# interstellar/zkvm

Hardware: AMD Instinct MI355X
Metric: ZkVM tx verifications/sec (batch) (higher is better)
Workload: dtype u32 limb pairs of radix-2^51 (v_mad_u64_u32)

## Files before the change

### zkvm_amd/csrc/kernels.hpp

```cpp
#pragma once
#include "curve.hpp"
#include "quad.hpp"
#include "sc_dev.hpp"

namespace zk {

constexpr uint32_t ENTRY_NEG = 1u << 31;
constexpr uint32_t ENTRY_DYN = 1u << 30;
constexpr uint32_t ENTRY_IDX = (1u << 30) - 1;
constexpr int NIELS_WORDS = 32;
constexpr int EXT_WORDS = 40;
constexpr int REDUCE_CHUNK = 64;
#ifndef ZK_REDUCE_CHUNK_BIG
#define ZK_REDUCE_CHUNK_BIG 16
#endif
constexpr int REDUCE_CHUNK_BIG = ZK_REDUCE_CHUNK_BIG;
constexpr int TABLE_WORDS = 24;
constexpr int TABLE_STRIDE = 32;

struct JobDesc {
  const uint32_t* dyn_scalars;
  const uint64_t* dyn_offsets;
  uint64_t n_dyn;
  const uint32_t* st_scalars;
// ... 871 lines not shown
  fe_mul(c4.T, p.T, fe_D2());
  store_ext(row, c4);
}

__global__ void __launch_bounds__(64)
k_small_tables(const uint32_t* __restrict__ dyn_scalars, const uint32_t* __restrict__ dyn_rows, uint64_t n,
               uint32_t* __restrict__ tbl , uint32_t* __restrict__ recoded ,
               uint32_t* __restrict__ status) {
  const uint64_t k = (uint64_t)blockIdx.x * 64 + threadIdx.x;
  if (k >= n) return;
  if (dyn_scalars) {
    const uint32_t* sc = dyn_scalars + 8 * k;
    if (sc[7] >> 31) atomicOr(&status[0], 2u);
    uint32_t carry = 0;
#pragma unroll
    for (int i = 0; i < 8; ++i) {
      const uint64_t v = (uint64_t)sc[i] + 0x88888888u + carry;
      recoded[8 * k + i] = (uint32_t)v;
      carry = (uint32_t)(v >> 32);
    }
  }
  ge_niels nq;
  load_niels(nq, dyn_rows + k * NIELS_WORDS);
  ge cur;
  ge_identity(cur);
  uint32_t* row = tbl + k * (SMALL_TBL * EXT_WORDS);
#pragma unroll 1
  for (int e = 0; e < SMALL_TBL; ++e) {
    ge_madd(cur, cur, nq, false);
    store_cached(row + e * EXT_WORDS, cur);
  }
}

__global__ void __launch_bounds__(256)
k_small_accumulate(const uint32_t* __restrict__ recoded, const uint64_t* __restrict__ dyn_offsets,
                   const uint32_t* __restrict__ tbl, uint32_t n_msm, uint32_t* __restrict__ window_sums,
                   uint32_t* __restrict__ window_nonempty) {
  extern __shared__ __attribute__((aligned(16))) uint32_t smem[];
  const uint32_t m = blockIdx.x;
  const int t = threadIdx.x & 63;
  const int part = threadIdx.x >> 6, parts = blockDim.x >> 6;
  const uint64_t k0 = dyn_offsets[m], k1 = dyn_offsets[m + 1];
  ge total;
  bool total_set = false;
#pragma unroll 1
  for (uint64_t k = k0 + part; k < k1; k += parts) {
    const uint32_t n4 = (recoded[8 * k + (t >> 3)] >> (4 * (t & 7))) & 15u;
    const int d = (t == 63 && n4 < 8u) ? (int)n4 + 8 : (int)n4 - 8;
    if (d != 0) {
      ge c4;
      load_ext(c4, tbl + (k * SMALL_TBL + (uint64_t)((d < 0 ? -d : d) - 1)) * EXT_WORDS);
      ge_cached c;
      c.YpX = c4.X; c.YmX = c4.Y; c.Z2 = c4.Z; c.T2d = c4.T;
      if (!total_set) { ge_identity(total); total_set = true; }
      ge_add_cached(total, total, c, d < 0);
    }
  }
  if (part > 0) {
    uint32_t* slot = smem + (uint32_t)(part - 1) * 41 * 64;
    slot[40 * 64 + t] = total_set ? 1u : 0u;
    if (total_set) {
#pragma unroll
      for (int q = 0; q < 10; ++q) {
        slot[q * 64 + t] = total.X.v[q]; slot[(10 + q) * 64 + t] = total.Y.v[q];
        slot[(20 + q) * 64 + t] = total.Z.v[q]; slot[(30 + q) * 64 + t] = total.T.v[q];
      }
    }
  }
  __syncthreads();
  if (part != 0) return;
#pragma unroll 1
  for (int o = 1; o < parts; ++o) {
    const uint32_t* slot = smem + (uint32_t)(o - 1) * 41 * 64;
    if (slot[40 * 64 + t]) {
      ge other;
#pragma unroll
      for (int q = 0; q < 10; ++q) {
        other.X.v[q] = slot[q * 64 + t]; other.Y.v[q] = slot[(10 + q) * 64 + t];
        other.Z.v[q] = slot[(20 + q) * 64 + t]; other.T.v[q] = slot[(30 + q) * 64 + t];
      }
      if (total_set) ge_add(total, total, other); else { total = other; total_set = true; }
    }
  }
  const uint64_t win = (uint64_t)m * 64 + t;
  window_nonempty[win] = total_set ? 1u : 0u;
  if (total_set) store_ext(window_sums + win * EXT_WORDS, total);
}

__global__ void __launch_bounds__(256)
k_msm_finish_quad(const uint32_t* __restrict__ window_sums, const uint32_t* __restrict__ window_nonempty,
                  const uint32_t* __restrict__ msm_fail, uint8_t* __restrict__ accept,
                  uint32_t* __restrict__ out_enc, uint32_t* __restrict__ out_ext, uint32_t n_msm, int w,
                  int n_windows, const uint32_t* __restrict__ sel_state, uint32_t sel_group) {
  const uint32_t g = blockIdx.x * blockDim.x + threadIdx.x;
  const int r = g & 3;
  const bool live = (g >> 2) < n_msm;
  const uint32_t m = live ? (g >> 2) : (n_msm - 1);
  if (sel_state && sel_state[m / sel_group] == 0) return;
  ge acc;
  ge_identity(acc);
  bool have = false;
  const uint64_t win0 = (uint64_t)m * n_windows;
  ge p;
  uint32_t ne = window_nonempty[win0 + n_windows - 1];
  load_ext(p, window_sums + (win0 + n_windows - 1) * EXT_WORDS);
  for (int t = n_windows - 1; t >= 0; --t) {
    ge pn;
    uint32_t nen = 0;
    if (t > 0) {
      nen = window_nonempty[win0 + t - 1];
      load_ext(pn, window_sums + (win0 + t - 1) * EXT_WORDS);
    }
    if (have) {
      for (int k = 0; k < w; ++k) quad_double(acc, r);
    }
    if (ne) {
      if (have) quad_add(acc, p, r); else { acc = p; have = true; }
    }
    if (t > 0) { p = pn; ne = nen; }
// ... 135 lines not shown
    ge_niels nq;
    niels_from_affine(nq, x, y);
    store_table_row(myrows + (uint64_t)d * TABLE_STRIDE, nq);
  }
}

__global__ void __launch_bounds__(256)
k_static_digits(const uint32_t* __restrict__ st_scalars, int16_t* __restrict__ digits, uint64_t n_static, int w,
                int W, uint32_t* __restrict__ status, const uint32_t* __restrict__ row_map ,
                const uint32_t* __restrict__ n_active , uint32_t rows_per_msm, uint32_t fold_small_negatives) {
  uint64_t k = (uint64_t)blockIdx.x * blockDim.x + threadIdx.x;
  if (k >= n_static) return;
  if (row_map) {
    const uint32_t slot = (uint32_t)(k / rows_per_msm);
    if (slot >= *n_active) return;
    k = (uint64_t)row_map[slot] * rows_per_msm + k % rows_per_msm;
  }
  const uint32_t* sc = st_scalars + 8 * k;
  if (sc[7] >> 31) atomicOr(&status[0], 2u);
  for (int t = 0; t < W; ++t) digits[(uint64_t)t * n_static + k] = 0;
  if (fold_small_negatives) {
    const uint32_t l[8] = ZK_SC_L;
    uint32_t v[8];
    uint64_t br = 0;
    for (int i = 0; i < 8; ++i) { const uint64_t d = (uint64_t)l[i] - sc[i] - br; v[i] = (uint32_t)d; br = (d >> 32) & 1; }
    uint32_t high = v[0] >> 14;
    for (int i = 1; i < 8; ++i) high |= v[i];
    if (br == 0 && high == 0 && v[0] != 0 && w >= 15) { digits[k] = (int16_t)(-(int)v[0]); return; }
  }
  for_each_digit(sc, w, W, [&](int t, int d) { digits[(uint64_t)t * n_static + k] = (int16_t)d; });
}

template <bool kSkipZeros>
__global__ void __launch_bounds__(256)
k_static_accumulate(const int16_t* __restrict__ digits, const uint64_t* __restrict__ st_offsets,
                    const uint32_t* __restrict__ st_index, const uint32_t* __restrict__ table, uint32_t n_set,
                    uint32_t H, int W, int P, uint32_t n_msm, uint64_t n_static, uint32_t* __restrict__ partials,
                    const uint32_t* __restrict__ row_map ,
                    const uint32_t* __restrict__ n_active ,
                    uint32_t interleave ) {
  const uint64_t lane = (uint64_t)blockIdx.x * blockDim.x + threadIdx.x;
  if (lane >= (uint64_t)n_msm * W * P) return;
  const uint32_t part = (uint32_t)(lane % P);
  uint32_t slot = (uint32_t)((lane / P) % n_msm);
  const uint32_t t = (uint32_t)(lane / ((uint64_t)P * n_msm));
  if (n_active && slot >= *n_active) return;
  if (interleave > 1) { const uint32_t per = n_msm / interleave; slot = (slot % per) * interleave + slot / per; }
  const uint32_t tx = row_map ? row_map[slot] : slot;
  const uint64_t k0 = st_offsets[tx], k1 = st_offsets[tx + 1];
  const int16_t* dig = digits + (uint64_t)t * n_static;
  const uint64_t tbase = (uint64_t)t * n_set;
  ge acc;
  ge_identity(acc);
  auto fetch = [&](uint64_t k, ge_niels& q, bool& neg, bool& any) {
    int d = dig[k];
    d = (d == -32768) ? 32768 : d;
    any = d != 0;
    const uint32_t idx = st_index ? st_index[k] : (uint32_t)(k - k0);
    const uint32_t mag = (uint32_t)(d < 0 ? -d : d);
    if (!kSkipZeros || any) load_table_row(q, table + ((tbase + idx) * H + (mag ? mag - 1 : 0)) * TABLE_STRIDE);
    if (!any) niels_identity(q);
    neg = d < 0;
  };
  uint64_t k = k0 + part;
  ge_niels cur, nxt;
  bool cur_neg = false, nxt_neg = false, cur_any = false, nxt_any = false;
  if (k < k1) fetch(k, cur, cur_neg, cur_any);
  while (k < k1) {
    const uint64_t kn = k + P;
    if (kn < k1) fetch(kn, nxt, nxt_neg, nxt_any);
    if (!kSkipZeros || __any(cur_any)) ge_madd(acc, acc, cur, cur_neg);
    cur = nxt; cur_neg = nxt_neg; cur_any = nxt_any;
    k = kn;
  }
  store_ext(partials + (((uint64_t)slot * W + t) * P + part) * EXT_WORDS, acc);
}

__device__ inline void static_combine_slot(const uint32_t* __restrict__ partials, uint32_t n_partials, const uint32_t* __restrict__ dyn_sum,
                                           const uint8_t* __restrict__ dyn_ok, uint32_t slot, uint32_t tx, int lane,
                                           uint8_t* __restrict__ accept, uint32_t* __restrict__ out_points) {
  ge acc;
  ge_identity(acc);
  for (uint32_t c = lane; c < n_partials; c += 64) {
    ge p;
    load_ext(p, partials + ((uint64_t)slot * n_partials + c) * EXT_WORDS);
    ge_add(acc, acc, p);
  }
  if (lane == 0 && dyn_sum) {
    ge p;
    load_ext(p, dyn_sum + (uint64_t)tx * EXT_WORDS);
    ge_add(acc, acc, p);
  }
#pragma unroll 1
  for (int delta = 32; delta >= 1; delta >>= 1) {
    ge other;
    shfl_down_ge(other, acc, delta);
    if (lane < delta) ge_add(acc, acc, other);
  }
  if (lane == 0) {
    accept[tx] = (ge_is_identity(acc) && (!dyn_ok || dyn_ok[tx])) ? 1 : 0;
    if (out_points) store_ext(out_points + (uint64_t)slot * EXT_WORDS, acc);
  }
}

constexpr uint32_t COMBINE_LANES = 8;

__global__ void __launch_bounds__(64)
k_static_combine(const uint32_t* __restrict__ partials, uint32_t n_partials, const uint32_t* __restrict__ dyn_sum,
                 const uint8_t* __restrict__ dyn_ok, const uint32_t* __restrict__ row_map,
                 const uint32_t* __restrict__ n_active, uint32_t n_slots, uint8_t* __restrict__ accept,
// ... 518 lines not shown
```

### zkvm_amd/csrc/zkgpu.hip

```cpp
#include "../../include/zkgpu.h"
#include "../../include/zkgpu_hooks.h"
#include "kernels.hpp"
#include "keccak.hpp"

#include <hip/hip_runtime.h>

#include <algorithm>
#include <chrono>
#include <cerrno>
#include <cstdio>
#include <cstring>
#include <functional>
#include <memory>
#include <mutex>
#include <string>
#include <map>
#include <atomic>
#include <dirent.h>
#include <sys/random.h>
#include <unistd.h>
#include <thread>
#include <type_traits>
#include <vector>

// ... 66 lines not shown
  int sync_rc = 0, reasons_src = 0;
  std::recursive_mutex mu;
  std::string last_error;
  Buffer in_scalars, in_points, in_offsets, in_st_scalars, in_st_index, in_st_offsets;
  Buffer dyn_rows, bins, block_sums, entries, buckets, partials, partial_flags, window_sums, window_flags;
  Buffer msm_fail, status, accept, bitmap, ok_bytes, values, uniform;
  Buffer digits, st_partials, dynsum, accept2, bin_order, class_count, part_hist, part_entries, part_lo, dec_scratch, heavy;
  Buffer small_tbl, recoded;
  Buffer grp_sc, grp_digits, grp_partials, grp_ok, row_map;
  Buffer grp_ws, grp_wf, grp_dyn;
  Buffer grp_fail, grp_fail_sum, rechk_pts;
  struct LastBatch { bool valid = false, has_prep = false; const zkgpu_pointset* ps = nullptr; std::vector<uint8_t> job, prep; bool mixed = false; uint64_t mx_groups = 0, mx_stmts = 0; } last;
  bool force_unresolved = false;
  uint64_t regroup_fallbacks = 0, mx_stats[4] = {0, 0, 0, 0};
  int group_size = 16;
  bool serial = false;
  int horner_mode = 0;
  std::atomic<uint32_t> last_failed_groups{0};
  hipEvent_t ev_dig = nullptr, ev_u = nullptr;
  Buffer prep_com, prep_proofs, prep_r, prep_pw, prep_ch, prep_wf, prep_dyn_sc, prep_dyn_pt, prep_st_sc;
  Buffer coal_com, coal_proofs, coal_r, tx_reason;
  Buffer ipa_lv, ipa_rv, ipa_cg, ipa_ch, ipa_w, ipa_u;
  Buffer pv_plan, pv_state, pv_in, pv_rows0, pv_rows1, pv_rows2, pv_rows3, pv_lay, pv_pts, pv_com, pv_ab, pv_proofs;
  int prover_mode = 0;
  int prover_slices = 0;
  std::vector<zkgpu_ctx*> pv_slices;
  std::vector<uint32_t> pv_plan_host;
  size_t pv_lay_batch = 0;
  Buffer prep_absorb, prep_raw, mx_tab, mx_st_index, prep_large, mx_grp_index;
  int locate_mode = 0;
  int transcript_mode = 0;
  int forced_parts = 0;
  int locate_parts = 0;
  int tail_mode = 0;
  void* pinned = nullptr;
  size_t pinned_cap = 0;
  void* pinned_in = nullptr;
  size_t pinned_in_cap = 0;
  bool profiling = false;
  std::vector<ProfEntry> prof;
  std::vector<std::pair<hipEvent_t, hipEvent_t>> ev_pool;
  std::vector<std::pair<int, int>> ev_used;
  size_t ev_next = 0;
  int forced_w = 0, last_w = 0;
  DecodeRoutes decode_routes;
  uint64_t last_adds = 0, tx_hashed_on_device = 0, tx_signed_on_device = 0;
};

namespace {
void quiesce_after_fault(zkgpu_ctx* c) {
  zk::fault::Suppress open;
  int prev = -1;
  (void)hipGetDevice(&prev);
  if (prev != c->device) (void)hipSetDevice(c->device);
  if (hipDeviceSynchronize() != hipSuccess) c->broken = true;
  (void)hipGetLastError();
  if (prev >= 0 && prev != c->device) (void)hipSetDevice(prev);
}

#define HIP_TRY(ctx, expr)                                                                  \
  do {                                                                                      \
    if ((ctx)->broken) {                                                                    \
      (ctx)->last_error = "an earlier device fault on this context could not be drained: the context is unusable"; \
      return ZKGPU_EHIP;                                                                    \
    }                                                                                       \
    hipError_t e__ = (expr);                                                                \
    if (e__ != hipSuccess) {                                                                \
// ... 622 lines not shown
  return pipe_tables(c, ps) && pipe_rows_fit(n_msm, n_dyn, n_static);
}

int pipe_enqueue(zkgpu_ctx* c, const Job& job, const zkgpu_pointset* ps, const PrepLaunch* prep) {
  static_assert(std::is_trivially_copyable<Job>::value && std::is_trivially_copyable<PrepLaunch>::value, "kept as bytes");
  {
    std::vector<uint8_t> jb(sizeof(Job)), pb(prep ? sizeof(PrepLaunch) : 0);
    memcpy(jb.data(), &job, sizeof(Job));
    if (prep) memcpy(pb.data(), prep, sizeof(PrepLaunch));
    c->last.job.swap(jb); c->last.prep.swap(pb);
    c->last.ps = ps; c->last.has_prep = prep != nullptr; c->last.valid = true; c->last.mixed = false;
  }
  const size_t B = job.n_msm;
  const size_t nbytes = (B + 7) / 8;
  hipStream_t L = c->stream_l, H1 = c->serial ? L : c->stream, H2 = c->serial ? L : c->stream2;
  const hipStream_t H3s = c->serial ? L : c->stream3;
  const int W = ps->tbl_W;
  int P = c->forced_parts;
  if (P <= 0) {
    P = (int)((131072 + B * W - 1) / (B * W));
    P = std::max(1, std::min(16, P));
  }
  const uint64_t n_lanes = (uint64_t)B * W * P;
  const uint32_t group = (prep && c->group_size > 1) ? (uint32_t)std::min<size_t>(c->group_size, B) : 1;
  const uint32_t n_groups = (uint32_t)((B + group - 1) / group);
  const uint32_t ns = prep ? prep->plan.sh.n_static : 0;
  const bool locate = group > 1 && (c->locate_mode >= 2 || (c->locate_mode == 0 && B >= LOCATE_MIN_BATCH));
  const bool spec = locate && c->locate_mode == 3;
  const uint32_t grp_rows = spec ? 2 * n_groups : n_groups;
  int Pg = 1;
  const int Pf = 32;
  const int Pl = c->locate_parts > 0 ? c->locate_parts : 32;
  if (group > 1) {
    Pg = (int)std::max<uint64_t>(1, std::min<uint64_t>(32, (65536 + (uint64_t)grp_rows * W - 1) / ((uint64_t)grp_rows * W)));
    TRY(ensure(c, c->grp_sc, (size_t)grp_rows * ns * 32));
    TRY(ensure(c, c->grp_digits, (size_t)grp_rows * ns * W * 2));
    TRY(ensure(c, c->grp_partials, (size_t)grp_rows * std::max<size_t>((size_t)W * std::max(Pg, locate && !spec ? Pl : 0), TAIL_THREADS) * EXT_WORDS * 4));
    TRY(ensure(c, c->grp_ok, n_groups));
    TRY(ensure(c, c->row_map, B * 4));
    TRY(ensure(c, c->grp_fail, (size_t)n_groups * 12));
    TRY(ensure(c, c->grp_fail_sum, (size_t)n_groups * EXT_WORDS * 4));
    TRY(ensure(c, c->grp_ws, (size_t)n_groups * 64 * EXT_WORDS * 4));
    TRY(ensure(c, c->grp_wf, (size_t)n_groups * 64 * 4));
    TRY(ensure(c, c->grp_dyn, (size_t)n_groups * EXT_WORDS * 4));
    TRY(ensure(c, c->rechk_pts, B * EXT_WORDS * 4));
  }
  TRY(ensure(c, c->accept, B));
  TRY(ensure(c, c->accept2, B));
  TRY(ensure(c, c->bitmap, nbytes));
  TRY(ensure_pinned(c, nbytes + 64 + (c->want_reasons ? B : 0)));
  TRY(ensure(c, c->status, 64));
  TRY(ensure(c, c->digits, std::max<uint64_t>(job.n_static, 1) * W * 2));
  TRY(ensure(c, c->st_partials, std::max<uint64_t>(n_lanes, group > 1 ? (uint64_t)B * std::max(W * Pf, TAIL_THREADS) : 0) * EXT_WORDS * 4));
  TRY(ensure(c, c->dynsum, B * EXT_WORDS * 4));
  TRY(ensure(c, c->dyn_rows, std::max<uint64_t>(job.n_dyn, 1) * NIELS_WORDS * 4));
  TRY(ensure(c, c->window_sums, (size_t)B * 64 * EXT_WORDS * 4));
  TRY(ensure(c, c->window_flags, (size_t)B * 64 * 4));
  TRY(ensure(c, c->msm_fail, (size_t)B * 4));
  TRY(ensure(c, c->small_tbl, std::max<uint64_t>(job.n_dyn, 1) * SMALL_TBL * EXT_WORDS * 4));
  TRY(ensure(c, c->recoded, std::max<uint64_t>(job.n_dyn, 1) * 32));
  c->last_w = 4;
  if (c->reserve_only) return ZKGPU_OK;
  const int phase = prep ? c->enqueue_phase : (int)zkgpu_ctx::ENQ_ALL;
  if (phase == zkgpu_ctx::ENQ_ALL || phase == zkgpu_ctx::ENQ_FRONT) {
  {
    Launch l(c, "k_batch_init", L);
    hipLaunchKernelGGL(k_batch_init, dim3(blocks_for(B, 256)), dim3(256), 0, L, (uint32_t*)c->status.p,
// ... 26 lines not shown
        hipLaunchKernelGGL(k_challenges, dim3((unsigned)B), dim3(128), (size_t)sh.n_ch * 32, L, sh, (const uint32_t*)c->prep_raw.p,
                           (const uint32_t*)c->prep_pw.p, prep->d_r, (uint32_t)B, (uint32_t*)c->prep_ch.p,
                           (uint32_t*)c->prep_wf.p, d.mono_chal, d.mono_pow, group > 1 ? 1u : 0u);
      }
    } else {
      Launch l(c, "k_transcript", L);
      hipLaunchKernelGGL(k_transcript, dim3(blocks_for(B, 64)), dim3(64), 0, L, sh, d.init, d.tape, d.n_ops, prep->d_com,
                         (const uint32_t*)c->prep_pw.p, prep->d_r, (uint32_t)B, (uint32_t*)c->prep_ch.p,
                         (uint32_t*)c->prep_wf.p, d.mono_chal, d.mono_pow, group > 1 ? 1u : 0u);
    }
  }
  HIP_TRY(c, hipEventRecord(c->ev_t, L));
  }
  if (phase == zkgpu_ctx::ENQ_FRONT) { HIP_TRY(c, hipGetLastError()); c->awaiting_back = true; return ZKGPU_OK; }
  if (prep && (phase == zkgpu_ctx::ENQ_ALL || phase == zkgpu_ctx::ENQ_MID)) {
    const PrepShape& sh = prep->plan.sh;
    HIP_TRY(c, hipStreamWaitEvent(H1, c->ev_u, 0));
    {
      Launch l(c, "k_points_tables", H1);
      hipLaunchKernelGGL(k_points_tables, dim3(blocks_for((uint64_t)B * sh.n_dyn, 256)), dim3(256), 0, H1, sh,
                         prep->d_com, (const uint32_t*)c->prep_pw.p, (uint32_t)B, (uint32_t*)c->small_tbl.p,
                         (uint32_t*)c->msm_fail.p, (unsigned long long*)((char*)c->status.p + 8));
    }
    HIP_TRY(c, hipEventRecord(c->ev_dig, H1));
  }
  if (phase == zkgpu_ctx::ENQ_MID) { HIP_TRY(c, hipGetLastError()); return ZKGPU_OK; }
  c->awaiting_back = false;
  if (prep) {
    HIP_TRY(c, hipStreamWaitEvent(H3s, c->ev_t, 0));
    TRY(prepare_launch(c, H3s, *prep, (uint32_t)B, false));
  }
  HIP_TRY(c, hipEventRecord(c->ev_p, prep ? H3s : L));
  HIP_TRY(c, hipStreamWaitEvent(H1, c->ev_p, 0));
  HIP_TRY(c, hipStreamWaitEvent(H2, c->ev_p, 0));
  uint32_t* n_recheck = (uint32_t*)((char*)c->status.p + 32);
  if (group > 1) {
    HIP_TRY(c, hipStreamWaitEvent(H2, c->ev_dig, 0));
    {
      Launch l(c, "k_group_scalars", H2);
      hipLaunchKernelGGL(k_group_scalars, dim3(blocks_for((uint64_t)n_groups * ns, 256)), dim3(256), 0, H2,
                         job.d_st_scalars, (uint32_t)B, ns, group, (uint32_t*)c->grp_sc.p, (int16_t*)c->grp_digits.p,
                         ps->tbl_w, W, (const uint32_t*)c->msm_fail.p, job.d_wellformed, spec ? 1u : 0u);
    }
    {
      Launch l(c, "k_static_accumulate", H2);
      hipLaunchKernelGGL(k_static_accumulate<false>, dim3(blocks_for((uint64_t)grp_rows * W * Pg, 256)), dim3(256), 0, H2,
                         (const int16_t*)c->grp_digits.p, job.d_st_offsets, job.d_st_index, (const uint32_t*)ps->table,
                         (uint32_t)ps->n, ps->tbl_H, W, Pg, grp_rows, (uint64_t)grp_rows * ns,
                         (uint32_t*)c->grp_partials.p, (const uint32_t*)nullptr, (const uint32_t*)nullptr, 1u);
    }
    HIP_TRY(c, hipEventRecord(c->ev_sa, H2));
  } else {
    {
      Launch l(c, "k_static_digits", H2);
      hipLaunchKernelGGL(k_static_digits, dim3(blocks_for(job.n_static, 256)), dim3(256), 0, H2, job.d_st_scalars,
                         (int16_t*)c->digits.p, job.n_static, ps->tbl_w, W, (uint32_t*)c->status.p,
                         (const uint32_t*)nullptr, (const uint32_t*)nullptr, 0u, 0u);
    }
    {
      Launch l(c, "k_static_accumulate", H2);
      hipLaunchKernelGGL(k_static_accumulate<false>, dim3(blocks_for(n_lanes, 256)), dim3(256), 0, H2,
                         (const int16_t*)c->digits.p, job.d_st_offsets, job.d_st_index, (const uint32_t*)ps->table,
                         (uint32_t)ps->n, ps->tbl_H, W, P, (uint32_t)B, job.n_static, (uint32_t*)c->st_partials.p,
                         (const uint32_t*)nullptr, (const uint32_t*)nullptr, 1u);
    }
    HIP_TRY(c, hipEventRecord(c->ev_sa, H2));
  }
  if (prep) {
    TRY(small_accumulate_launch(c, job, H1));
  } else {
    decompress_launch(c, job, H1);
    TRY(small_msm_launch(c, job, H1));
  }
  HIP_TRY(c, hipEventRecord(c->ev_sm, H1));
  HIP_TRY(c, hipStreamWaitEvent(L, c->ev_sm, 0));
  zkgpu_ctx* root = c->parent ? c->parent : c;
  const bool group_first = group > 1 && !spec && (c->horner_mode == 2 || (c->horner_mode == 0 && root->last_failed_groups.load() == 0));
  if (group_first) {
    {
      Launch l(c, "k_group_windows", L);
      hipLaunchKernelGGL(k_group_windows, dim3(blocks_for((uint64_t)n_groups * 64, 256)), dim3(256), 0, L,
                         (const uint32_t*)c->window_sums.p, (const uint32_t*)c->window_flags.p, (const uint32_t*)c->msm_fail.p,
                         job.d_wellformed, (uint32_t)B, group, 64u, (uint32_t*)c->grp_ws.p, (uint32_t*)c->grp_wf.p);
    }
    Launch l(c, "k_msm_finish_quad", L);
    hipLaunchKernelGGL(k_msm_finish_quad, dim3(blocks_for(4 * (uint64_t)n_groups, 256)), dim3(256), 0, L,
                       (const uint32_t*)c->grp_ws.p, (const uint32_t*)c->grp_wf.p, (const uint32_t*)nullptr, (uint8_t*)nullptr,
                       (uint32_t*)nullptr, (uint32_t*)c->grp_dyn.p, n_groups, 4, 64, (const uint32_t*)nullptr, 0u);
  } else {
    Launch l(c, "k_msm_finish_quad", L);
    hipLaunchKernelGGL(k_msm_finish_quad, dim3(blocks_for(4 * B, 256)), dim3(256), 0, L,
                       (const uint32_t*)c->window_sums.p, (const uint32_t*)c->window_flags.p,
                       (const uint32_t*)c->msm_fail.p, (uint8_t*)c->accept.p, (uint32_t*)nullptr,
                       (uint32_t*)c->dynsum.p, (uint32_t)B, 4, 64, (const uint32_t*)nullptr, 0u);
  }
  HIP_TRY(c, hipStreamWaitEvent(L, c->ev_sa, 0));
  if (group > 1) {
    uint32_t* n_fail = (uint32_t*)((char*)c->status.p + 36);
    uint32_t* fail_list = (uint32_t*)c->grp_fail.p;
    uint32_t* cand = fail_list + n_groups;
    uint32_t* grp_state = cand + n_groups;
    {
      Launch l(c, "k_group_combine", L);
      hipLaunchKernelGGL(spec ? k_group_combine<true> : k_group_combine<false>, dim3(n_groups), dim3(256), 0, L, (const uint32_t*)c->grp_partials.p,
                         (uint32_t)(W * Pg), group_first ? (const uint32_t*)c->grp_dyn.p : (const uint32_t*)nullptr,
                         (const uint32_t*)c->dynsum.p, (const uint32_t*)c->msm_fail.p,
                         job.d_wellformed, (uint32_t)B, group, (uint8_t*)c->accept2.p, grp_state, fail_list,
                         (uint32_t*)c->grp_fail_sum.p, n_fail, job.d_st_scalars, ns, (uint32_t*)c->grp_sc.p,
                         (int16_t*)c->grp_digits.p, ps->tbl_w, W, spec ? 2u : locate ? 1u : 0u, (uint32_t*)c->row_map.p, n_recheck, cand,
                         (int16_t*)c->digits.p);
    }
    if (group_first) {
      Launch l(c, "k_msm_finish_quad", L);
      hipLaunchKernelGGL(k_msm_finish_quad, dim3(blocks_for(4 * B, 256)), dim3(256), 0, L,
                         (const uint32_t*)c->window_sums.p, (const uint32_t*)c->window_flags.p,
                         (const uint32_t*)c->msm_fail.p, (uint8_t*)c->accept.p, (uint32_t*)nullptr,
                         (uint32_t*)c->dynsum.p, (uint32_t)B, 4, 64, (const uint32_t*)grp_state, group);
    }
    const bool fused_tail = c->tail_mode == 0;
    if (locate && !spec && fused_tail) {
      Launch l(c, "k_locate_fused", L);
      hipLaunchKernelGGL(k_locate_fused, dim3(n_groups), dim3(LOCATE_THREADS), 0, L, (const int16_t*)c->grp_digits.p, job.d_st_offsets, job.d_st_index,
                         (const uint32_t*)ps->table, (uint32_t)ps->n, ps->tbl_H, n_groups, (uint32_t*)c->grp_partials.p,
                         (const uint32_t*)c->dynsum.p, (const uint32_t*)c->msm_fail.p, job.d_wellformed, (uint32_t)B, group,
                         (const uint32_t*)fail_list, (const uint32_t*)n_fail, (const uint32_t*)c->grp_fail_sum.p,
                         (uint32_t*)c->row_map.p, n_recheck, cand, job.d_st_scalars, ns, (int16_t*)c->digits.p, ps->tbl_w, W);
    }
    if (locate && !spec && !fused_tail) {
      Launch l(c, "k_static_accumulate", L);
// ... 234 lines not shown
}

int ctx_create(int device, zkgpu_ctx* parent, zkgpu_ctx** out, int aux = 0) {
  zkgpu_ctx* c = new zkgpu_ctx();
  c->device = device;
  int prio_least = 0, prio_greatest = 0;
  (void)hipDeviceGetStreamPriorityRange(&prio_least, &prio_greatest);
  bool ok = true;
  if (parent) {
    constexpr int lanes = STREAM_SETS;
    ++parent->n_forks;
    const int set = (int)(++parent->fork_seq % lanes);
    c->parent = parent;
    while (ok && (int)parent->lane_streams.size() < 3 * (lanes - 1)) {
      hipStream_t st = nullptr;
      const int which = (int)parent->lane_streams.size() % 3;
      ok = hipStreamCreateWithPriority(&st, hipStreamNonBlocking, which == 1 ? prio_least : prio_greatest) == hipSuccess;
      if (ok) parent->lane_streams.push_back(st);
    }
    if (ok && set > 0) {
      c->stream = parent->lane_streams[3 * (set - 1)];
      c->stream2 = parent->lane_streams[3 * (set - 1) + 1];
      c->stream3 = parent->lane_streams[3 * (set - 1) + 2];
    } else {
      c->stream = parent->stream;
      c->stream2 = parent->stream2;
      c->stream3 = parent->stream3;
    }
    c->owns_streams = false;
    c->group_size = parent->group_size;
    c->transcript_mode = parent->transcript_mode;
    c->locate_mode = parent->locate_mode;
    c->locate_parts = parent->locate_parts;
    c->tail_mode = parent->tail_mode;
    c->horner_mode = parent->horner_mode;
  } else if (aux == 2) {
    ok = hipStreamCreateWithPriority(&c->stream, hipStreamNonBlocking, prio_greatest) == hipSuccess;
  } else if (aux) {
    ok = hipStreamCreateWithPriority(&c->stream, hipStreamNonBlocking, prio_greatest) == hipSuccess &&
         hipStreamCreateWithPriority(&c->stream2, hipStreamNonBlocking, prio_greatest) == hipSuccess;
  } else {
    ok = hipStreamCreateWithPriority(&c->stream, hipStreamNonBlocking, prio_greatest) == hipSuccess &&
         hipStreamCreateWithPriority(&c->stream2, hipStreamNonBlocking, prio_least) == hipSuccess &&
         hipStreamCreateWithPriority(&c->stream3, hipStreamNonBlocking, prio_greatest) == hipSuccess;
    std::vector<hipStream_t> rejected;
    for (int attempt = 0; ok && attempt < 6; ++attempt) {
      const int ov = streams_overlap(c->stream, c->stream2);
      c->pair_overlaps = ov;
      if (ov != 0) break;
      rejected.push_back(c->stream2);
      c->stream2 = nullptr;
      ok = hipStreamCreateWithPriority(&c->stream2, hipStreamNonBlocking, prio_least) == hipSuccess;
    }
    for (hipStream_t st : rejected) (void)hipStreamDestroy(st);
  }
  if (!aux) ok = ok && hipStreamCreateWithPriority(&c->stream_l, hipStreamNonBlocking, prio_greatest) == hipSuccess;
  hipEvent_t* evs[] = {&c->ev_fork, &c->ev_join, &c->ev_t, &c->ev_p, &c->ev_sm, &c->ev_sa, &c->ev_done, &c->ev_dig, &c->ev_u};
  for (hipEvent_t* e : evs) ok = ok && hipEventCreateWithFlags(e, hipEventDisableTiming) == hipSuccess;
  if (!ok) { if (parent) --parent->n_forks; delete c; return ZKGPU_EHIP; }
  *out = c;
  return ZKGPU_OK;
}
}

int zkgpu_runtime_hint(char* buf, size_t cap) {
  static const char kHint[] = "GPU_MAX_HW_QUEUES=2";
  if (buf && cap) { strncpy(buf, kHint, cap - 1); buf[cap - 1] = 0; }
// ... 253 lines not shown
  }
  e = hipGetLastError();
  if (e == hipSuccess) e = hipStreamSynchronize(c->stream);
  if (c->profiling) prof_collect(c);
  (void)hipFree(base);
  (void)hipFree(tmp);
  if (e != hipSuccess) { (void)hipFree(table); c->last_error = hipGetErrorString(e); return ZKGPU_EHIP; }
  ps->table = table; ps->tbl_w = w; ps->tbl_W = W; ps->tbl_H = H;
  return ZKGPU_OK;
}

size_t zkgpu_pointset_table_bytes(const zkgpu_pointset* ps) {
  return (ps && ps->table) ? (size_t)ps->tbl_W * ps->n * ps->tbl_H * TABLE_STRIDE * 4 : 0;
}

static long long debug_read_buffers(zkgpu_ctx* c, const char* what, void* out, size_t bytes) {
  if (!c || !what || !out) return ZKGPU_EINVAL;
  std::lock_guard<std::recursive_mutex> lk(c->mu);
  DeviceGuard g(c->device);
  const std::string w(what);
#ifdef ZK_PREP_STAMPS
  if (w == "prep_stamps") {
    const size_t n = std::min(bytes, sizeof(unsigned long long) * 256 * 2 * zk::PREP_STAMP_SLOTS);
    if (hipDeviceSynchronize() != hipSuccess || hipMemcpyFromSymbol(out, HIP_SYMBOL(zk::g_prep_stamps), n) != hipSuccess) return ZKGPU_EHIP;
    return (long long)n;
  }
#endif
  if (w == "prover_slices") {
    if (bytes < 4) return ZKGPU_EINVAL;
    const uint32_t n = (uint32_t)c->last_prover_slices;
    memcpy(out, &n, 4);
    return 4;
  }
  const Buffer* b = w == "challenges" ? &c->prep_ch : w == "static_scalars" ? &c->prep_st_sc :
                    w == "dyn_scalars" ? &c->prep_dyn_sc : w == "dyn_points" ? &c->prep_dyn_pt : nullptr;
  if (!b || !b->p) return ZKGPU_EINVAL;
  const size_t n = std::min(bytes, b->cap);
  if (hipDeviceSynchronize() != hipSuccess || hipMemcpy(out, b->p, n, hipMemcpyDeviceToHost) != hipSuccess) return ZKGPU_EHIP;
  return (long long)n;
}

int zkgpu_set_serial(zkgpu_ctx* c, int on) {
  if (!c) return ZKGPU_EINVAL;
  std::lock_guard<std::recursive_mutex> lk(c->mu);
  c->serial = on != 0;
  return ZKGPU_OK;
}

int zkgpu_set_prover_mode(zkgpu_ctx* c, int mode) {
  if (!c || mode < 0 || (mode > 1 && (mode < 17 || mode > 24))) return ZKGPU_EINVAL;
  std::lock_guard<std::recursive_mutex> lk(c->mu);
  c->prover_mode = mode > 1 ? 0 : mode;
  c->prover_slices = mode > 1 ? mode - 16 : 0;
  return ZKGPU_OK;
}

int zkgpu_set_horner_mode(zkgpu_ctx* c, int mode) {
  if (!c || mode < 0 || mode > 2) return ZKGPU_EINVAL;
  std::lock_guard<std::recursive_mutex> lk(c->mu);
  c->horner_mode = mode;
  return ZKGPU_OK;
}

int zkgpu_set_transcript_mode(zkgpu_ctx* c, int mode) {
  if (!c || mode < 0 || mode > 2) return ZKGPU_EINVAL;
  std::lock_guard<std::recursive_mutex> lk(c->mu);
  c->transcript_mode = mode;
  return ZKGPU_OK;
// ... 28 lines not shown
  HIP_TRY(c, hipMemcpyAsync(out, c->values.p, 32 * n, hipMemcpyDeviceToHost, c->stream));
  HIP_TRY(c, hipStreamSynchronize(c->stream));
  return ZKGPU_OK;
}

int zkgpu_set_locate_mode(zkgpu_ctx* c, int mode) {
  if (!c || mode < 0 || mode > 3) return ZKGPU_EINVAL;
  std::lock_guard<std::recursive_mutex> lk(c->mu);
  c->locate_mode = mode;
  return ZKGPU_OK;
}

long long zkgpu_debug_force_regroup(zkgpu_ctx* c, int on) {
  if (!c) return ZKGPU_EINVAL;
  std::lock_guard<std::recursive_mutex> lk(c->mu);
  c->force_unresolved = on != 0;
  return (long long)c->regroup_fallbacks;
}

int zkgpu_set_group_size(zkgpu_ctx* c, int group) {
  if (!c || group < 1 || group > 64) return ZKGPU_EINVAL;
  std::lock_guard<std::recursive_mutex> lk(c->mu);
  c->group_size = group;
  return ZKGPU_OK;
}

int zkgpu_set_static_parts(zkgpu_ctx* c, int parts) {
  if (!c || parts < 0 || parts > 64) return ZKGPU_EINVAL;
  c->forced_parts = parts;
  return ZKGPU_OK;
}

int zkgpu_set_tail_mode(zkgpu_ctx* c, int mode) {
  if (!c || mode < 0 || mode > 1) return ZKGPU_EINVAL;
  std::lock_guard<std::recursive_mutex> lk(c->mu);
  c->tail_mode = mode;
  return ZKGPU_OK;
}

int zkgpu_set_locate_parts(zkgpu_ctx* c, int parts) {
  if (!c || parts < 0 || parts > 64) return ZKGPU_EINVAL;
  std::lock_guard<std::recursive_mutex> lk(c->mu);
  c->locate_parts = parts;
  return ZKGPU_OK;
}

int zkgpu_verify_batch_ps_dev(zkgpu_ctx* c, const zkgpu_pointset* ps, size_t batch, const void* d_dyn_scalars,
                              const void* d_dyn_points, const void* d_dyn_offsets, size_t n_dyn,
                              const void* d_static_scalars, const void* d_static_index,
                              const void* d_static_offsets, size_t n_static, uint8_t* accept_bitmap) {
  if (!c || !ps || ps->ctx->device != c->device || !accept_bitmap || batch >= (1ull << 31)) return ZKGPU_EINVAL;
  if (batch && (!d_dyn_offsets || !d_static_offsets)) return ZKGPU_EINVAL;
  if ((n_dyn && (!d_dyn_scalars || !d_dyn_points)) || (n_static && !d_static_scalars)) return ZKGPU_EINVAL;
  std::lock_guard<std::recursive_mutex> lk(c->mu);
  memset(accept_bitmap, 0, (batch + 7) / 8);
  TRY(refuse_if_pending(c));
  DeviceGuard g(c->device);
  Job job;
  job.d_dyn_scalars = (const uint32_t*)d_dyn_scalars;
  job.d_dyn_points = (const uint32_t*)d_dyn_points;
  job.d_dyn_offsets = (const uint64_t*)d_dyn_offsets;
  job.n_dyn = n_dyn;
  job.d_st_scalars = (const uint32_t*)d_static_scalars;
  job.d_st_index = (const uint32_t*)d_static_index;
  job.d_st_offsets = (const uint64_t*)d_static_offsets;
  job.n_static = n_static;
  job.d_static_rows = ps->rows;
  job.n_msm = (uint32_t)batch;
  int rc = (ps->table && n_static) ? batch_device_tables(c, job, ps, accept_bitmap) : batch_device(c, job, accept_bitmap);
// ... 1760 lines not shown
```

### zkvm_amd/native.py

```python
from __future__ import annotations

import ctypes as C
import os
import struct
import weakref
from typing import Dict, List, Optional, Sequence, Tuple

HERE = os.path.dirname(os.path.abspath(__file__))
_LIB = None

OK, EINVAL, EINVALID_POINT, EHIP, ENOMEM, ENODEVICE, ENOCOMM = 0, -1, -2, -3, -4, -5, -6


class ZkGpuError(RuntimeError):
    def __init__(self, code: int, msg: str, index: Optional[int] = None):
        super().__init__(f"zkgpu error {code}: {msg}" + (f" (index {index})" if index is not None else ""))
        self.code = code
        self.index = index


def lib_path() -> str:
    return os.environ.get("ZKGPU_LIB") or os.path.join(HERE, "lib", "libzkgpu.so")


# ... 444 lines not shown
        return ok.raw[:n]

    def profile(self, on: bool) -> None:
        self.lib.zkgpu_profile_enable(self.h, 1 if on else 0)

    def profile_reset(self) -> None:
        self.lib.zkgpu_profile_reset(self.h)

    def profile_read(self) -> Dict[str, Tuple[int, float]]:
        out = {}
        for i in range(self.lib.zkgpu_profile_count(self.h)):
            name, n, ms = C.c_char_p(), C.c_uint64(), C.c_double()
            self.lib.zkgpu_profile_get(self.h, i, C.byref(name), C.byref(n), C.byref(ms))
            out[name.value.decode()] = (int(n.value), float(ms.value))
        return out

    def debug_read(self, what: str, nbytes: int) -> bytes:
        buf = C.create_string_buffer(max(nbytes, 1))
        n = int(self.lib.zkgpu_debug_read(self.h, what.encode(), buf, nbytes))
        if n < 0:
            raise ZkGpuError(n, "zkgpu_debug_read(%s)" % what)
        return buf.raw[:n]

    def last_window_bits(self) -> int:
        return int(self.lib.zkgpu_last_window_bits(self.h))

    def set_static_parts(self, parts: int) -> None:
        self._check(self.lib.zkgpu_set_static_parts(self.h, parts))

    def set_locate_parts(self, parts: int) -> None:
        self._check(self.lib.zkgpu_set_locate_parts(self.h, parts))

    def set_tail_mode(self, mode: int) -> None:
        self._check(self.lib.zkgpu_set_tail_mode(self.h, mode))

    def set_window_bits(self, w: int) -> None:
        self._check(self.lib.zkgpu_set_window_bits(self.h, w))


class R1csDescStruct(C.Structure):
    _fields_ = [("transcript_label", C.c_char_p), ("n_commitments", C.c_uint32), ("n_multipliers_phase1", C.c_uint32),
                ("n_multipliers", C.c_uint32), ("n_challenges", C.c_uint32), ("challenge_labels", C.POINTER(C.c_char_p)),
                ("n_constraints", C.c_uint32), ("term_offsets", C.POINTER(C.c_uint64)), ("term_var_kind", C.POINTER(C.c_uint8)),
                ("term_var_index", C.POINTER(C.c_uint32)), ("term_coeff", C.c_char_p), ("term_challenge", C.POINTER(C.c_int32)),
                ("term_power", C.POINTER(C.c_uint32))]


class R1csDescription:
    KIND_COMMITTED, KIND_LEFT, KIND_RIGHT, KIND_OUT, KIND_ONE = range(5)
    L = 2**252 + 27742317777372353535851937790883648493

    def __init__(self, label: bytes, n_commitments: int, n_phase1: int, n_multipliers: int, challenge_labels, constraints):
        self.label, self.m, self.n1, self.n = label, n_commitments, n_phase1, n_multipliers
        self.challenge_labels = list(challenge_labels)
        self.constraints = constraints
        offs, kinds, idx, coeff, chal, power = [0], [], [], bytearray(), [], []
        for con in constraints:
            for (k, i, c, ch, pw) in con:
                kinds.append(k); idx.append(i); coeff += int(c % self.L).to_bytes(32, "little"); chal.append(ch); power.append(pw)
            offs.append(len(kinds))
        nt = max(len(kinds), 1)
        self._keep = ((C.c_char_p * max(len(self.challenge_labels), 1))(*self.challenge_labels), (C.c_uint64 * len(offs))(*offs),
                      (C.c_uint8 * nt)(*kinds), (C.c_uint32 * nt)(*idx), bytes(coeff), (C.c_int32 * nt)(*chal), (C.c_uint32 * nt)(*power))
        k = self._keep
        self.struct = R1csDescStruct(label, self.m, self.n1, self.n, len(self.challenge_labels), k[0], len(constraints), k[1], k[2], k[3],
                                     k[4], k[5], k[6])

# ... 52 lines not shown
```

Measured before the change: 3.349 million.

## Fuse static accumulate and small dynamic accumulate into one kernel launch

Adds k_accumulate_fused, which gives the grouped static bucket accumulation and the small-table dynamic window accumulation separate ranges of block indices in one grid on stream H1. Both previously ran as separate kernels on streams H2 and H1 joined by events. The fused path is on by default in the grouped, prepared, non-serial case. It removes one launch and the cross-stream event waits, and lets both workloads fill the GPU together. In exchange, the static part now uses the dynamic kernel's block size and shared-memory allocation, and loses overlap with other work previously queued on H2.

```diff
diff --git a/zkvm_amd/csrc/kernels.hpp b/zkvm_amd/csrc/kernels.hpp
--- a/zkvm_amd/csrc/kernels.hpp
+++ b/zkvm_amd/csrc/kernels.hpp
@@ -927,12 +927,9 @@
   }
 }
 
-__global__ void __launch_bounds__(256)
-k_small_accumulate(const uint32_t* __restrict__ recoded, const uint64_t* __restrict__ dyn_offsets,
-                   const uint32_t* __restrict__ tbl, uint32_t n_msm, uint32_t* __restrict__ window_sums,
-                   uint32_t* __restrict__ window_nonempty) {
-  extern __shared__ __attribute__((aligned(16))) uint32_t smem[];
-  const uint32_t m = blockIdx.x;
+__device__ __forceinline__ void small_accumulate_msm(uint32_t m, const uint32_t* __restrict__ recoded, const uint64_t* __restrict__ dyn_offsets,
+                                                     const uint32_t* __restrict__ tbl, uint32_t* __restrict__ window_sums,
+                                                     uint32_t* __restrict__ window_nonempty, uint32_t* smem) {
   const int t = threadIdx.x & 63;
   const int part = threadIdx.x >> 6, parts = blockDim.x >> 6;
   const uint64_t k0 = dyn_offsets[m], k1 = dyn_offsets[m + 1];
@@ -980,6 +977,14 @@
   const uint64_t win = (uint64_t)m * 64 + t;
   window_nonempty[win] = total_set ? 1u : 0u;
   if (total_set) store_ext(window_sums + win * EXT_WORDS, total);
+}
+
+__global__ void __launch_bounds__(256)
+k_small_accumulate(const uint32_t* __restrict__ recoded, const uint64_t* __restrict__ dyn_offsets,
+                   const uint32_t* __restrict__ tbl, uint32_t n_msm, uint32_t* __restrict__ window_sums,
+                   uint32_t* __restrict__ window_nonempty) {
+  extern __shared__ __attribute__((aligned(16))) uint32_t smem[];
+  small_accumulate_msm(blockIdx.x, recoded, dyn_offsets, tbl, window_sums, window_nonempty, smem);
 }
 
 __global__ void __launch_bounds__(256)
@@ -1181,14 +1186,10 @@
 }
 
 template <bool kSkipZeros>
-__global__ void __launch_bounds__(256)
-k_static_accumulate(const int16_t* __restrict__ digits, const uint64_t* __restrict__ st_offsets,
-                    const uint32_t* __restrict__ st_index, const uint32_t* __restrict__ table, uint32_t n_set,
-                    uint32_t H, int W, int P, uint32_t n_msm, uint64_t n_static, uint32_t* __restrict__ partials,
-                    const uint32_t* __restrict__ row_map ,
-                    const uint32_t* __restrict__ n_active ,
-                    uint32_t interleave ) {
-  const uint64_t lane = (uint64_t)blockIdx.x * blockDim.x + threadIdx.x;
+__device__ __forceinline__ void static_accumulate_lane(uint64_t lane, const int16_t* __restrict__ digits, const uint64_t* __restrict__ st_offsets,
+                                                       const uint32_t* __restrict__ st_index, const uint32_t* __restrict__ table, uint32_t n_set,
+                                                       uint32_t H, int W, int P, uint32_t n_msm, uint64_t n_static, uint32_t* __restrict__ partials,
+                                                       const uint32_t* __restrict__ row_map, const uint32_t* __restrict__ n_active, uint32_t interleave) {
   if (lane >= (uint64_t)n_msm * W * P) return;
   const uint32_t part = (uint32_t)(lane % P);
   uint32_t slot = (uint32_t)((lane / P) % n_msm);
@@ -1225,6 +1226,49 @@
   store_ext(partials + (((uint64_t)slot * W + t) * P + part) * EXT_WORDS, acc);
 }
 
+template <bool kSkipZeros>
+__global__ void __launch_bounds__(256)
+k_static_accumulate(const int16_t* __restrict__ digits, const uint64_t* __restrict__ st_offsets,
+                    const uint32_t* __restrict__ st_index, const uint32_t* __restrict__ table, uint32_t n_set,
+                    uint32_t H, int W, int P, uint32_t n_msm, uint64_t n_static, uint32_t* __restrict__ partials,
+                    const uint32_t* __restrict__ row_map ,
+                    const uint32_t* __restrict__ n_active ,
+                    uint32_t interleave ) {
+  static_accumulate_lane<kSkipZeros>((uint64_t)blockIdx.x * blockDim.x + threadIdx.x, digits, st_offsets, st_index, table, n_set, H, W, P,
+                                     n_msm, n_static, partials, row_map, n_active, interleave);
+}
+
+__global__ void __launch_bounds__(256)
+k_accumulate_fused(uint32_t n_static_blocks, const int16_t* __restrict__ digits, const uint64_t* __restrict__ st_offsets,
+                   const uint32_t* __restrict__ st_index, const uint32_t* __restrict__ table, uint32_t n_set, uint32_t H, int W,
+                   int P, uint32_t n_rows, uint64_t n_static, uint32_t* __restrict__ partials,
+                   const uint32_t* __restrict__ recoded, const uint64_t* __restrict__ dyn_offsets,
+                   const uint32_t* __restrict__ tbl, uint32_t* __restrict__ window_sums, uint32_t* __restrict__ window_nonempty) {
+  extern __shared__ __attribute__((aligned(16))) uint32_t smem[];
+  if (blockIdx.x < n_static_blocks) {
+    static_accumulate_lane<false>((uint64_t)blockIdx.x * blockDim.x + threadIdx.x, digits, st_offsets, st_index, table, n_set, H, W, P,
+                                  n_rows, n_static, partials, nullptr, nullptr, 1u);
+    return;
+  }
+  small_accumulate_msm(blockIdx.x - n_static_blocks, recoded, dyn_offsets, tbl, window_sums, window_nonempty, smem);
+}
+
+#ifndef ZK_GROUP_LANES
+#define ZK_GROUP_LANES 65536
+#endif
+constexpr uint64_t GROUP_LANES = ZK_GROUP_LANES;
+
+inline void accumulate_fused_launch(hipStream_t st, uint32_t n_msm, int parts, const int16_t* digits, const uint64_t* st_offsets,
+                                    const uint32_t* st_index, const uint32_t* table, uint32_t n_set, uint32_t H, int W, int P,
+                                    uint32_t n_rows, uint64_t n_static, uint32_t* partials, const uint32_t* recoded,
+                                    const uint64_t* dyn_offsets, const uint32_t* tbl, uint32_t* window_sums, uint32_t* window_nonempty) {
+  const uint32_t block = 64u * (uint32_t)parts;
+  const uint32_t n_static_blocks = (uint32_t)(((uint64_t)n_rows * W * P + block - 1) / block);
+  hipLaunchKernelGGL(k_accumulate_fused, dim3(n_static_blocks + n_msm), dim3(block), (size_t)(parts - 1) * 41 * 64 * 4, st, n_static_blocks,
+                     digits, st_offsets, st_index, table, n_set, H, W, P, n_rows, n_static, partials, recoded, dyn_offsets, tbl, window_sums,
+                     window_nonempty);
+}
+
 __device__ inline void static_combine_slot(const uint32_t* __restrict__ partials, uint32_t n_partials, const uint32_t* __restrict__ dyn_sum,
                                            const uint8_t* __restrict__ dyn_ok, uint32_t slot, uint32_t tx, int lane,
                                            uint8_t* __restrict__ accept, uint32_t* __restrict__ out_points) {
diff --git a/zkvm_amd/csrc/zkgpu.hip b/zkvm_amd/csrc/zkgpu.hip
--- a/zkvm_amd/csrc/zkgpu.hip
+++ b/zkvm_amd/csrc/zkgpu.hip
@@ -122,7 +122,7 @@
   int transcript_mode = 0;
   int forced_parts = 0;
   int locate_parts = 0;
-  int tail_mode = 0;
+  int tail_mode = 0, accumulate_mode = 0;
   void* pinned = nullptr;
   size_t pinned_cap = 0;
   void* pinned_in = nullptr;
@@ -811,7 +811,7 @@
   const int Pf = 32;
   const int Pl = c->locate_parts > 0 ? c->locate_parts : 32;
   if (group > 1) {
-    Pg = (int)std::max<uint64_t>(1, std::min<uint64_t>(32, (65536 + (uint64_t)grp_rows * W - 1) / ((uint64_t)grp_rows * W)));
+    Pg = c->forced_parts > 0 ? std::min(32, c->forced_parts) : (int)std::max<uint64_t>(1, std::min<uint64_t>(32, (GROUP_LANES + (uint64_t)grp_rows * W - 1) / ((uint64_t)grp_rows * W)));
     TRY(ensure(c, c->grp_sc, (size_t)grp_rows * ns * 32));
     TRY(ensure(c, c->grp_digits, (size_t)grp_rows * ns * W * 2));
     TRY(ensure(c, c->grp_partials, (size_t)grp_rows * std::max<size_t>((size_t)W * std::max(Pg, locate && !spec ? Pl : 0), TAIL_THREADS) * EXT_WORDS * 4));
@@ -904,24 +904,28 @@
   }
   HIP_TRY(c, hipEventRecord(c->ev_p, prep ? H3s : L));
   HIP_TRY(c, hipStreamWaitEvent(H1, c->ev_p, 0));
-  HIP_TRY(c, hipStreamWaitEvent(H2, c->ev_p, 0));
+  const bool fused_acc = group > 1 && prep && c->accumulate_mode == 0 && !c->serial; const hipStream_t Hg = fused_acc ? H1 : H2;
+  if (!fused_acc) HIP_TRY(c, hipStreamWaitEvent(H2, c->ev_p, 0));
   uint32_t* n_recheck = (uint32_t*)((char*)c->status.p + 32);
+  auto static_sums = [&](const void* dig, int parts, uint32_t rows, uint64_t n_st, void* out) {
+    Launch l(c, "k_static_accumulate", H2);
+    hipLaunchKernelGGL(k_static_accumulate<false>, dim3(blocks_for((uint64_t)rows * W * parts, 256)), dim3(256), 0, H2, (const int16_t*)dig, job.d_st_offsets, job.d_st_index,
+                       (const uint32_t*)ps->table, (uint32_t)ps->n, ps->tbl_H, W, parts, rows, n_st, (uint32_t*)out, (const uint32_t*)nullptr, (const uint32_t*)nullptr, 1u);
+  };
   if (group > 1) {
-    HIP_TRY(c, hipStreamWaitEvent(H2, c->ev_dig, 0));
+    if (!fused_acc) HIP_TRY(c, hipStreamWaitEvent(H2, c->ev_dig, 0));
     {
-      Launch l(c, "k_group_scalars", H2);
-      hipLaunchKernelGGL(k_group_scalars, dim3(blocks_for((uint64_t)n_groups * ns, 256)), dim3(256), 0, H2,
+      Launch l(c, "k_group_scalars", Hg);
+      hipLaunchKernelGGL(k_group_scalars, dim3(blocks_for((uint64_t)n_groups * ns, 256)), dim3(256), 0, Hg,
                          job.d_st_scalars, (uint32_t)B, ns, group, (uint32_t*)c->grp_sc.p, (int16_t*)c->grp_digits.p,
                          ps->tbl_w, W, (const uint32_t*)c->msm_fail.p, job.d_wellformed, spec ? 1u : 0u);
     }
-    {
-      Launch l(c, "k_static_accumulate", H2);
-      hipLaunchKernelGGL(k_static_accumulate<false>, dim3(blocks_for((uint64_t)grp_rows * W * Pg, 256)), dim3(256), 0, H2,
-                         (const int16_t*)c->grp_digits.p, job.d_st_offsets, job.d_st_index, (const uint32_t*)ps->table,
-                         (uint32_t)ps->n, ps->tbl_H, W, Pg, grp_rows, (uint64_t)grp_rows * ns,
-                         (uint32_t*)c->grp_partials.p, (const uint32_t*)nullptr, (const uint32_t*)nullptr, 1u);
-    }
-    HIP_TRY(c, hipEventRecord(c->ev_sa, H2));
+    if (fused_acc) {
+      Launch l(c, "k_accumulate_fused", H1);
+      accumulate_fused_launch(H1, (uint32_t)B, small_parts(B), (const int16_t*)c->grp_digits.p, job.d_st_offsets, job.d_st_index, (const uint32_t*)ps->table, (uint32_t)ps->n,
+                              ps->tbl_H, W, Pg, grp_rows, (uint64_t)grp_rows * ns, (uint32_t*)c->grp_partials.p, (const uint32_t*)c->recoded.p, job.d_dyn_offsets,
+                              (const uint32_t*)c->small_tbl.p, (uint32_t*)c->window_sums.p, (uint32_t*)c->window_flags.p);
+    } else static_sums(c->grp_digits.p, Pg, grp_rows, (uint64_t)grp_rows * ns, c->grp_partials.p);
   } else {
     {
       Launch l(c, "k_static_digits", H2);
@@ -929,17 +933,11 @@
                          (int16_t*)c->digits.p, job.n_static, ps->tbl_w, W, (uint32_t*)c->status.p,
                          (const uint32_t*)nullptr, (const uint32_t*)nullptr, 0u, 0u);
     }
-    {
-      Launch l(c, "k_static_accumulate", H2);
-      hipLaunchKernelGGL(k_static_accumulate<false>, dim3(blocks_for(n_lanes, 256)), dim3(256), 0, H2,
-                         (const int16_t*)c->digits.p, job.d_st_offsets, job.d_st_index, (const uint32_t*)ps->table,
-                         (uint32_t)ps->n, ps->tbl_H, W, P, (uint32_t)B, job.n_static, (uint32_t*)c->st_partials.p,
-                         (const uint32_t*)nullptr, (const uint32_t*)nullptr, 1u);
-    }
-    HIP_TRY(c, hipEventRecord(c->ev_sa, H2));
-  }
+    static_sums(c->digits.p, P, (uint32_t)B, job.n_static, c->st_partials.p);
+  }
+  if (!fused_acc) HIP_TRY(c, hipEventRecord(c->ev_sa, H2));
   if (prep) {
-    TRY(small_accumulate_launch(c, job, H1));
+    if (!fused_acc) TRY(small_accumulate_launch(c, job, H1));
   } else {
     decompress_launch(c, job, H1);
     TRY(small_msm_launch(c, job, H1));
@@ -966,7 +964,7 @@
                        (const uint32_t*)c->msm_fail.p, (uint8_t*)c->accept.p, (uint32_t*)nullptr,
                        (uint32_t*)c->dynsum.p, (uint32_t)B, 4, 64, (const uint32_t*)nullptr, 0u);
   }
-  HIP_TRY(c, hipStreamWaitEvent(L, c->ev_sa, 0));
+  if (!fused_acc) HIP_TRY(c, hipStreamWaitEvent(L, c->ev_sa, 0));
   if (group > 1) {
     uint32_t* n_fail = (uint32_t*)((char*)c->status.p + 36);
     uint32_t* fail_list = (uint32_t*)c->grp_fail.p;
@@ -1267,7 +1265,7 @@
     c->transcript_mode = parent->transcript_mode;
     c->locate_mode = parent->locate_mode;
     c->locate_parts = parent->locate_parts;
-    c->tail_mode = parent->tail_mode;
+    c->tail_mode = parent->tail_mode; c->accumulate_mode = parent->accumulate_mode;
     c->horner_mode = parent->horner_mode;
   } else if (aux == 2) {
     ok = hipStreamCreateWithPriority(&c->stream, hipStreamNonBlocking, prio_greatest) == hipSuccess;
@@ -1587,8 +1585,8 @@
     memcpy(out, &n, 4);
     return 4;
   }
-  const Buffer* b = w == "challenges" ? &c->prep_ch : w == "static_scalars" ? &c->prep_st_sc :
-                    w == "dyn_scalars" ? &c->prep_dyn_sc : w == "dyn_points" ? &c->prep_dyn_pt : nullptr;
+  const Buffer* b = w == "challenges" ? &c->prep_ch : w == "static_scalars" ? &c->prep_st_sc : w == "dyn_scalars" ? &c->prep_dyn_sc : w == "dyn_points" ? &c->prep_dyn_pt :
+                    w == "window_sums" ? &c->window_sums : w == "window_flags" ? &c->window_flags : w == "grp_partials" ? &c->grp_partials : nullptr;
   if (!b || !b->p) return ZKGPU_EINVAL;
   const size_t n = std::min(bytes, b->cap);
   if (hipDeviceSynchronize() != hipSuccess || hipMemcpy(out, b->p, n, hipMemcpyDeviceToHost) != hipSuccess) return ZKGPU_EHIP;
@@ -1683,9 +1681,9 @@
 }
 
 int zkgpu_set_tail_mode(zkgpu_ctx* c, int mode) {
-  if (!c || mode < 0 || mode > 1) return ZKGPU_EINVAL;
-  std::lock_guard<std::recursive_mutex> lk(c->mu);
-  c->tail_mode = mode;
+  if (!c || mode < 0 || mode > 3) return ZKGPU_EINVAL;
+  std::lock_guard<std::recursive_mutex> lk(c->mu);
+  c->tail_mode = mode & 1; c->accumulate_mode = mode >> 1;
   return ZKGPU_OK;
 }
 
diff --git a/zkvm_amd/native.py b/zkvm_amd/native.py
--- a/zkvm_amd/native.py
+++ b/zkvm_amd/native.py
@@ -500,7 +500,14 @@
         self._check(self.lib.zkgpu_set_locate_parts(self.h, parts))
 
     def set_tail_mode(self, mode: int) -> None:
-        self._check(self.lib.zkgpu_set_tail_mode(self.h, mode))
+        self._tail_mode = mode & 1
+        self._check(self.lib.zkgpu_set_tail_mode(self.h, self._tail_mode | getattr(self, "_accumulate_mode", 0) << 1))
+
+    def set_accumulate_mode(self, mode: int) -> None:
+        if mode not in (0, 1):
+            raise ZkGpuError(EINVAL, "accumulate mode %r" % (mode,))
+        self._accumulate_mode = mode
+        self._check(self.lib.zkgpu_set_tail_mode(self.h, getattr(self, "_tail_mode", 0) | mode << 1))
 
     def set_window_bits(self, w: int) -> None:
         self._check(self.lib.zkgpu_set_window_bits(self.h, w))
```

Result: no change. 3.325 million (-0.7%).
